# xqz-u/contrast-gan-3D

Measured on NVIDIA B200. Metric: patch_pairs_per_sec_gd_train_step, higher is better.
Workload: dtype bf16

## Files before the change

### contrast_gan_3d_b200/csrc/conv_tc_prog.cu

```cuda
#include "conv_tc_prog_kernel.cuh"

namespace cg {

extern template int prog_launch_ks<1>(ProgPlan &, const ProgLaunchArgs &);
extern template int prog_launch_ks<2>(ProgPlan &, const ProgLaunchArgs &);
extern template int prog_launch_ks<4>(ProgPlan &, const ProgLaunchArgs &);
extern template int prog_launch_ks<8>(ProgPlan &, const ProgLaunchArgs &);

__global__ void repack_prog_kernel(const bf16 *__restrict__ wp, bf16 *__restrict__ wb, int Cb, int Cs, int scatter,
                                   const __grid_constant__ ProgPlan p) {
  const int K = p.paired ? 16 : p.Cin, N = p.Nmma, nh = p.pair ? 2 : 1, Nl = N / nh;
  const int64_t total = (int64_t)p.nbt * K * N;
  for (int64_t i = blockIdx.x * (int64_t)blockDim.x + threadIdx.x; i < total; i += (int64_t)gridDim.x * blockDim.x) {
    const int c8 = (int)(i & 7);
    int64_t t = i >> 3;
    const int nl = (int)(t % Nl); t /= Nl;
    const int cc = (int)(t % (K >> 3)); t /= (K >> 3);
    const int tile = (int)(t % p.nbt);
    const int n = (int)(t / p.nbt) * Nl + nl;
    const int nn = p.stack ? n % p.N : n;
    const int tap = p.stack ? p.tile_phase_tap[tile][n / p.N] : (p.paired ? p.tile_tap[tile][cc] : tile);
    const int ci = p.paired ? c8 : cc * 8 + c8;
    bf16 v = __float2bfloat16_rn(0.f);
    if (nn < p.Nout && tap >= 0) {
// ... 113 lines not shown
            if (nt >= kMaxTaps) return false;
            ProgTap T{};
            T.row_shift = (uint16_t)((oy - offmin) * p.Zh + (oz - offmin));
            T.btile = (uint8_t)nt;
            T.acc = 0; T.first = first ? 1 : 0;
            first = false;
            for (int ph = 0; ph < 8; ++ph) p.tile_phase_tap[nt][ph] = taps8[ph];
            p.taps[nt++] = T; E.ntaps++;
          }
        if (E.ntaps == 0) continue;
        if (ne >= kMaxEntries) return false;
        p.entries[ne++] = E;
      }
      p.nacc = 8;
      p.nentries = ne;
      p.ntaps = nt;
      return true;
    }
    bool seen[8] = {false, false, false, false, false, false, false, false};
    for (int xo = offmin; xo <= offmax; ++xo) {
      ProgEntry E{};
      E.cx = (int8_t)xo; E.cy = (int8_t)offmin; E.cz = (int8_t)offmin;
      E.tap0 = (uint8_t)nt; E.ntaps = 0;
      for (int px = 0; px < 2; ++px)
        for (int dx = 0; dx < k; ++dx) {
          if (((px + 1 - dx) & 1) || (px + 1 - dx) / 2 != xo) continue;
          for (int py = 0; py < 2; ++py)
            for (int dy = 0; dy < k; ++dy) {
              if ((py + 1 - dy) & 1) continue;
              for (int pz = 0; pz < 2; ++pz)
                for (int dz = 0; dz < k; ++dz) {
                  if ((pz + 1 - dz) & 1) continue;
                  if (nt >= kMaxTaps) return false;
                  const int oy = (py + 1 - dy) / 2, oz = (pz + 1 - dz) / 2;
                  ProgTap T{};
                  T.row_shift = (uint16_t)((oy - offmin) * p.Zh + (oz - offmin));
                  T.btile = (uint8_t)((dx * k + dy) * k + dz);
                  T.acc = (uint8_t)((px * 2 + py) * 2 + pz);
                  T.first = seen[T.acc] ? 0 : 1;
                  seen[T.acc] = true;
                  p.taps[nt++] = T; E.ntaps++;
                }
            }
        }
      if (E.ntaps == 0) continue;
      if (ne >= kMaxEntries) return false;
      p.entries[ne++] = E;
    }
    p.nacc = 8;
  }
  p.nentries = ne;
  p.ntaps = nt;
  return true;
}

static bool plan_prog_split(const cgan3d_conv_geom &g, int scatter, ProgPlan &best, int nsplit);

static bool plan_prog(const cgan3d_conv_geom &g, int scatter, ProgPlan &best, int *nsplit_out = nullptr) {
  for (int ns = 1; ns <= 4; ns *= 2)
    if (plan_prog_split(g, scatter, best, ns)) {
      if (nsplit_out) *nsplit_out = ns;
      return true;
    }
  return false;
}

static bool plan_prog_split(const cgan3d_conv_geom &g, int scatter, ProgPlan &best, int nsplit) {
  if (g.stride != 2 || g.pad != 1 || (g.k != 3 && g.k != 4)) return false;
  const int Cin = scatter ? g.Cs : g.Cb, Nfull = scatter ? g.Cb : g.Cs;
  if (Nfull % nsplit || (nsplit > 1 && (Nfull / nsplit) % 16)) return false;
  const int Nout = Nfull / nsplit;
  const int paired = (!scatter && Cin == 8) ? 1 : 0;
  if (!paired && Cin != 16 && Cin != 32 && Cin != 64 && Cin != 128) return false;
  if (Nout % 8 || Nout < 8 || Nout > 256 || (Nout > 8 && Nout % 16)) return false;
  const int N = Nout < 16 ? 16 : Nout;
  const int nacc = scatter ? 8 : 1;
  if (scatter && (g.Xb > 2 * g.Xs || g.Yb > 2 * g.Ys || g.Zb > 2 * g.Zs)) return false;
  const int halo = (scatter && g.k == 4) ? 2 : 1;
  const int taps = g.k * g.k * g.k;
  ProgPlan p{};
  p.B = g.B; p.Xg = g.Xs; p.Yg = g.Ys; p.Zg = g.Zs;
  p.Xo = scatter ? g.Xb : g.Xs; p.Yo = scatter ? g.Yb : g.Ys; p.Zo = scatter ? g.Zb : g.Zs;
  p.Cin = Cin; p.N = N; p.nacc = nacc; p.Nout = Nout; p.paired = paired; p.out_pitch = Nfull; p.out_c0 = 0;
  p.in_scale = scatter ? 1 : 2; p.out_scale = scatter ? 2 : 1;
  p.nbt = paired ? taps / 2 + (g.k == 3 ? 9 : 0) : taps;
  p.btile_bytes = (uint32_t)(paired ? 16 : Cin) * N * 2;
  p.Nmma = N; p.acc_stride = 0; p.mt_stride = N;
  const bool pair_base = paired || Cin <= 64;
  p.pair = (pair_base && N % 32 == 0) ? 1 : 0;
  if (p.pair) p.btile_bytes /= 2;
  if (scatter && 8 * N <= 256) {
    const int ncombo = g.k == 3 ? 8 : 27;
    const uint32_t tile = (uint32_t)Cin * 8 * N * 2 / (pair_base ? 2 : 1);
    if ((ncombo * tile + 1023) / 1024 * 1024 + 40000 <= kSmemLimitProg) {
      p.stack = 1; p.Nmma = 8 * N; p.nbt = ncombo; p.btile_bytes = tile; p.pair = pair_base ? 1 : 0;
    }
  }
  const uint32_t b_total = (p.nbt * p.btile_bytes + 1023) / 1024 * 1024;
  if (b_total + 40000 > kSmemLimitProg) return false;
  const bool zpair = !scatter && !paired && (Cin == 16 || Cin == 32) && g.k == 3 && g.Zb % 2 == 0;
  p.zpair = zpair ? 1 : 0;
  const int a_swz = zpair ? 4 * Cin : ((!paired && Cin <= 64) ? 2 * Cin : 0);
  double best_score = 0;
  bool found = false;
  for (int nzt = 1; nzt <= 4; ++nzt) {
    const int Zt = (p.Zg + nzt - 1) / nzt, Zh = Zt + halo;
    if (2 * (Zh - 1) + 1 > 256) continue;
    for (int Yt = 1; Yt <= p.Yg; ++Yt) {
      const int Yh = Yt + halo;
      if (2 * (Yh - 1) + 1 > 256) break;
      const int mt = (Yt * Zh + 127) / 128;
      if (mt > 4 || 2 * nacc * mt * N > 512) break;
      const int rows_alloc = ((mt * 128 + halo * Zh + halo) + 7) / 8 * 8;
      if (rows_alloc > 16383 || Yh * Zh > rows_alloc) continue;
      const uint32_t slot = a_swz ? ((uint32_t)rows_alloc * a_swz + 1023) / 1024 * 1024 : (uint32_t)(paired ? 1 : Cin / 8) * rows_alloc * 16;
      const int nslots = (int)mn<uint32_t>(8, (kSmemLimitProg - b_total - 512) / slot);
      if (nslots < 3) break;
      const int nslabs = (p.Yg + Yt - 1) / Yt;
      const double eff = (double)p.Yg * p.Zg / ((double)nslabs * nzt * mt * 128);
      const double halo_cost = (double)(Yh * Zh) / (Yt * Zt);
      const double score = eff / (0.5 + 0.5 * halo_cost);
      if (score > best_score + 1e-9) {
        best_score = score; found = true;
        best = p;
        best.nzt = nzt; best.Zt = Zt; best.Zh = Zh; best.Yt = Yt; best.Yh = Yh; best.nslabs = nslabs; best.mtiles = mt;
        best.rows_alloc = rows_alloc; best.slot_bytes = slot; best.nslots = nslots;
      }
    }
  }
  if (!found) return false;
  ProgPlan &q = best;
  const int es = q.in_scale;
  q.a_swz = a_swz;
  if (q.stack) { q.acc_stride = q.N; q.mt_stride = 8 * q.N; }
  else { q.acc_stride = q.mtiles * q.N; q.mt_stride = q.N; }
  q.box_bytes = (a_swz ? (uint32_t)a_swz : 16u) * q.Zh * q.Yh;
  (void)es;
  uint32_t cols = 32;
  while (cols < (uint32_t)(2 * nacc * q.mtiles * N)) cols <<= 1;
  q.tmem_cols = cols;
  q.smem_bytes = b_total + q.nslots * q.slot_bytes + 512;
  q.a_lbo_bytes = paired ? 16u : (uint32_t)q.rows_alloc * 16;
  if (!build_program(g, scatter, q)) return false;
  if (paired || q.stack) {
    if ((uint32_t)q.ntaps * q.btile_bytes > b_total) return false;
    q.nbt = q.ntaps;
  }
  return true;
}

bool tc_prog_supported(const cgan3d_conv_geom &g, int dtype, int op) {
  if (dtype != CGAN3D_BF16 || (op != 0 && op != 1)) return false;
  ProgPlan p;
  return plan_prog(g, op, p);
}

size_t tc_prog_workspace_bytes(const cgan3d_conv_geom &g, int dtype, int op) {
  if (dtype != CGAN3D_BF16 || (op != 0 && op != 1)) return 0;
  ProgPlan p;
  int nsplit = 1;
  if (!plan_prog(g, op, p, &nsplit)) return 0;
  return (((size_t)p.nbt * p.btile_bytes * (p.pair ? 2 : 1) + 255) / 256 * 256) * nsplit + 256;
}

bool tc_prog_fuses_bnstats(const cgan3d_conv_geom &g, int scatter) {
  ProgPlan p;
  return plan_prog(g, scatter, p) && p.Nout <= 64;
}

int tc_prog_run(const cgan3d_conv_geom &g, int scatter, const void *in, const void *wp, void *outp, void *ws, size_t ws_bytes,
                cudaStream_t st, double *bn_sums) {
  ProgPlan p;
  int nsplit = 1;
  if (!plan_prog(g, scatter, p, &nsplit)) return fail(CGAN3D_E_UNSUPPORTED, "tcgen05 strided conv: no tiling for this shape");
  const size_t part_bytes = ((size_t)p.nbt * p.btile_bytes * (p.pair ? 2 : 1) + 255) / 256 * 256;
  const size_t need = part_bytes * nsplit;
  if (ws == nullptr || ws_bytes < need) return fail(CGAN3D_E_WORKSPACE, "tcgen05 strided conv: workspace %zu < %zu", ws_bytes, need);
  if ((reinterpret_cast<uintptr_t>(in) & 15) || (reinterpret_cast<uintptr_t>(outp) & 15) || (reinterpret_cast<uintptr_t>(ws) & 15))
    return fail(CGAN3D_E_ARG, "tcgen05 strided conv: pointers must be 16-byte aligned");
  EncodeTiledFn enc = tc_encode_fn();
  if (!enc) return fail(CGAN3D_E_UNSUPPORTED, "cuTensorMapEncodeTiled not available");
  const int Xi = scatter ? g.Xs : g.Xb, Yi = scatter ? g.Ys : g.Yb, Zi = scatter ? g.Zs : g.Zb, Ci = p.Cin;
  if ((reinterpret_cast<uintptr_t>(outp) & 15) || (p.Nout * 2) % 16 || (p.out_pitch * 2) % 16) return fail(CGAN3D_E_ARG, "tcgen05 strided conv: output rows must be 16-byte aligned");
  const int es = p.in_scale;
  CUtensorMap tm;
  const cuuint64_t zp = p.zpair ? 2 : 1;
  const cuuint64_t gdim[5] = {(cuuint64_t)Ci * zp, (cuuint64_t)Zi / zp, (cuuint64_t)Yi, (cuuint64_t)Xi, (cuuint64_t)g.B};
  const cuuint64_t gstr[4] = {(cuuint64_t)Ci * 2 * zp, (cuuint64_t)Zi * Ci * 2, (cuuint64_t)Yi * Zi * Ci * 2,
                              (cuuint64_t)Xi * Yi * Zi * Ci * 2};
  const cuuint32_t box[5] = {(cuuint32_t)(p.a_swz ? Ci * (int)zp : 8), (cuuint32_t)(p.zpair ? p.Zh : es * (p.Zh - 1) + 1),
                             (cuuint32_t)(es * (p.Yh - 1) + 1), 1, 1};
  const cuuint32_t estr[5] = {1, (cuuint32_t)(p.zpair ? 1 : es), (cuuint32_t)es, 1, 1};
  const CUtensorMapSwizzle swz = p.a_swz == 128 ? CU_TENSOR_MAP_SWIZZLE_128B
                                 : (p.a_swz == 64 ? CU_TENSOR_MAP_SWIZZLE_64B : (p.a_swz == 32 ? CU_TENSOR_MAP_SWIZZLE_32B : CU_TENSOR_MAP_SWIZZLE_NONE));
  CUresult r = enc(&tm, CU_TENSOR_MAP_DATA_TYPE_BFLOAT16, 5, const_cast<void *>(in), gdim, gstr, box, estr,
                   CU_TENSOR_MAP_INTERLEAVE_NONE, swz, CU_TENSOR_MAP_L2_PROMOTION_L2_128B, CU_TENSOR_MAP_FLOAT_OOB_FILL_NONE);
  if (r != CUDA_SUCCESS) return fail(CGAN3D_E_SHAPE, "cuTensorMapEncodeTiled (strided) failed with %d", (int)r);
  const long long total = (long long)p.B * p.nzt * p.nslabs * p.Xg;
  const int grid = p.pair ? 2 * (int)mn<long long>((total + 1) / 2, (long long)(num_sms() / 2)) : (int)mn<long long>(total, (long long)num_sms());
  if (bn_sums && p.Nout > 64) return fail(CGAN3D_E_UNSUPPORTED, "tcgen05 strided conv: fused BatchNorm statistics need <= 64 channels per launch");
  ProgLaunchArgs la{};
  la.tm = tm; la.g = g; la.scatter = scatter; la.nsplit = nsplit; la.grid = grid; la.wp = wp; la.outp = outp; la.ws = ws;
  la.part_bytes = part_bytes; la.bn_sums = bn_sums; la.st = st; la.enc = enc;
  switch (p.paired ? 1 : (p.Cin >> 4)) {
    case 1: return prog_launch_ks<1>(p, la);
    case 2: return prog_launch_ks<2>(p, la);
    case 4: return prog_launch_ks<4>(p, la);
    case 8: return prog_launch_ks<8>(p, la);
    default: return fail(CGAN3D_E_UNSUPPORTED, "tcgen05 strided conv: Cin must be 16, 32, 64 or 128");
  }
}

}
```

### contrast_gan_3d_b200/csrc/conv_tc_prog_kernel.cuh

```cuda
#pragma once
#include "common.cuh"
#include "conv_internal.cuh"
#include "tc_common.cuh"

namespace cg {

using bf16 = __nv_bfloat16;

constexpr int kMaxEntries = 16, kMaxTaps = 64;
constexpr uint32_t kSmemLimitProg = 232448 - 1024;

struct ProgTap {
  uint16_t row_shift;
  uint8_t btile;
  uint8_t acc;
  uint8_t first;
  uint8_t khalf;
  uint8_t pad[2];
};
struct ProgEntry {
  int8_t cx, cy, cz;
  uint8_t ntaps, tap0;
  uint8_t pad[3];
};
struct ProgPlan {
  int B, Xg, Yg, Zg;
  int Xo, Yo, Zo;
  int Cin, N, nacc;
  int Nout;
  int out_pitch, out_c0;
  int paired;
  uint32_t a_lbo_bytes;
  int a_swz;
  int in_scale;
  int out_scale;
  int Zt, nzt, Zh, Yt, nslabs, Yh;
  int mtiles, rows_alloc, nslots, nbt;
  int nentries, ntaps;
  uint32_t slot_bytes, btile_bytes, box_bytes, tmem_cols, smem_bytes;
  ProgEntry entries[kMaxEntries];
  ProgTap taps[kMaxTaps];
  int8_t tile_tap[kMaxTaps][2];
  int stack;
  int Nmma;
  int acc_stride, mt_stride;
  int8_t tile_phase_tap[kMaxTaps][8];
  int pair;
  int zpair;
};

template <int KSTEPS, int MT, int STATS, bool PAIR>
__global__ void __launch_bounds__(192, 1)
conv_prog_tc_kernel(const __grid_constant__ CUtensorMap tmA, const __grid_constant__ CUtensorMap tmW, const bf16 *__restrict__ wB,
                    bf16 *__restrict__ out, const __grid_constant__ ProgPlan p, double *__restrict__ bn_sums) {
  extern __shared__ __align__(1024) uint8_t smem[];
  uint8_t *bres = smem;
  uint8_t *ring = bres + (((size_t)p.nbt * p.btile_bytes + 1023) & ~(size_t)1023);
  uint64_t *bars = reinterpret_cast<uint64_t *>(ring + (size_t)p.nslots * p.slot_bytes);
  uint64_t *b_ready = bars, *s_full = bars + 1, *s_empty = s_full + p.nslots;
  uint64_t *tm_full = s_empty + p.nslots, *tm_empty = tm_full + 2;
  uint32_t *tmem_ptr = reinterpret_cast<uint32_t *>(tm_empty + 2);
  const int warp = threadIdx.x >> 5, lane = threadIdx.x & 31;

  if (threadIdx.x == 0) {
    tc::mbar_init(b_ready, 1);
    for (int i = 0; i < p.nslots; ++i) { tc::mbar_init(&s_full[i], 1); tc::mbar_init(&s_empty[i], 1); }
    for (int i = 0; i < 2; ++i) { tc::mbar_init(&tm_full[i], 1); tc::mbar_init(&tm_empty[i], PAIR ? 8 : 4); }
    tc::fence_barrier_init();
  }
  const uint32_t cta_rank = PAIR ? tc::cluster_ctarank() : 0u;
  if constexpr (PAIR) {
    __syncthreads();
    tc::cluster_sync();
  }
  if (warp == 5) {
    if constexpr (PAIR) { tc::tmem_alloc2(tmem_ptr, p.tmem_cols); tc::tmem_relinquish2(); }
    else { tc::tmem_alloc(tmem_ptr, p.tmem_cols); tc::tmem_relinquish(); }
  }
  tc::tc_fence_before();
  __syncthreads();
  if constexpr (PAIR) tc::cluster_sync();
  tc::tc_fence_after();
  const uint32_t tmem_base = *tmem_ptr;

  const long long total_steps = (long long)p.B * p.nzt * p.nslabs * p.Xg;
  const long long total = PAIR ? (total_steps + 1) / 2 : total_steps;
  const int nblk = PAIR ? (int)gridDim.x >> 1 : (int)gridDim.x, blk = PAIR ? (int)blockIdx.x >> 1 : (int)blockIdx.x;
  const int s_begin = (int)(total * blk / nblk), s_end = (int)(total * (blk + 1) / nblk);
  const int kch = (p.paired || p.a_swz) ? 1 : (p.Cin >> 3);
  auto decode = [&](int st, int &b, int &z0, int &zlen, int &y0, int &ylen, int &x) -> bool {
    bool live = true;
    if constexpr (PAIR) {
      st = 2 * st + (int)cta_rank;
      if (st >= total_steps) { st = (int)total_steps - 1; live = false; }
    }
    x = st % p.Xg; st /= p.Xg;
    const int sl = st % p.nslabs; st /= p.nslabs;
    const int zt = st % p.nzt;
    b = st / p.nzt;
    y0 = sl * p.Yt; ylen = min(p.Yt, p.Yg - y0);
    z0 = zt * p.Zt; zlen = min(p.Zt, p.Zg - z0);
    return live;
  };

  if (warp == 4) {
    if (lane == 0) {
      tc::tma_prefetch_desc(&tmA);
      if constexpr (PAIR) {
        tc::tma_prefetch_desc(&tmW);
        if (cta_rank == 0) tc::mbar_expect_tx(b_ready, 2u * (uint32_t)p.nbt * p.btile_bytes);
        const int trows = (int)(p.btile_bytes >> 8);
        for (int t = 0; t < p.nbt; ++t)
          tc::tma_load_2d_2cta(bres + (size_t)t * p.btile_bytes, &tmW, b_ready, 0, ((int)cta_rank * p.nbt + t) * trows);
      } else {
        tc::mbar_expect_tx(b_ready, (uint32_t)p.nbt * p.btile_bytes);
        for (int t = 0; t < p.nbt; ++t)
          tc::bulk_g2s(bres + (size_t)t * p.btile_bytes, reinterpret_cast<const uint8_t *>(wB) + (size_t)t * p.btile_bytes,
                       p.btile_bytes, b_ready);
      }
      uint32_t e = 0;
      for (int st = s_begin; st < s_end; ++st) {
        int b, z0, zlen, y0, ylen, x;
        decode(st, b, z0, zlen, y0, ylen, x);
        for (int en = 0; en < p.nentries; ++en, ++e) {
          const ProgEntry &E = p.entries[en];
          const uint32_t slot = e % p.nslots, use = e / p.nslots;
          if (use > 0) tc::mbar_wait(&s_empty[slot], (use - 1) & 1);
          uint8_t *dst = ring + (size_t)slot * p.slot_bytes;
          const int cz = (p.zpair ? z0 : p.in_scale * z0) + E.cz, cy = p.in_scale * y0 + E.cy, cx = p.in_scale * x + E.cx;
          if constexpr (PAIR) {
            if (cta_rank == 0) tc::mbar_expect_tx(&s_full[slot], 2 * p.box_bytes);
            tc::tma_load_5d_2cta(dst, &tmA, &s_full[slot], 0, cz, cy, cx, b);
            continue;
          }
          tc::mbar_expect_tx(&s_full[slot], p.box_bytes * kch);
          if (p.a_swz) {
            tc::tma_load_5d(dst, &tmA, &s_full[slot], 0, cz, cy, cx, b);
          } else {
            for (int cc = 0; cc < kch; ++cc)
              tc::tma_load_5d(dst + (size_t)cc * p.rows_alloc * 16, &tmA, &s_full[slot], cc * 8, cz, cy, cx, b);
          }
        }
      }
    }
  } else if (warp == 5 && cta_rank != 0) {
  } else if (warp == 5) {
    const bool leader = tc::elect_one();
    const uint32_t idesc = tc::make_idesc_bf16(PAIR ? 256 : 128, p.Nmma, 0, 0);
    const uint32_t ring_u32 = tc::smem_u32(ring), b_u32 = tc::smem_u32(bres);
    const uint32_t a_lbo = p.a_lbo_bytes, b_lbo = (uint32_t)(PAIR ? p.Nmma >> 1 : p.Nmma) * 16;
    auto commit = [&](uint64_t *bar) {
      if constexpr (PAIR) tc::umma_commit_2cta(bar, 3);
      else tc::umma_commit(bar);
    };
    const uint32_t a_row = p.a_swz ? (uint32_t)p.a_swz >> 4 : 1u;
    const uint64_t a_hi = p.a_swz ? tc::make_desc_sw(0, 8u * p.a_swz, (uint32_t)p.a_swz) : tc::make_desc(0, a_lbo, 128);
    const uint64_t b_hi = tc::make_desc(0, b_lbo, 128);
    const uint32_t a_kstep = p.a_swz ? 2u : (2 * a_lbo) >> 4, b_kstep = (2 * b_lbo) >> 4;
    tc::mbar_wait(b_ready, 0);
    tc::tc_fence_after();
    uint32_t e = 0, acc = 0;
    for (int st = s_begin; st < s_end; ++st, ++acc) {
      const uint32_t q = acc & 1, uq = acc >> 1;
      if (uq > 0) tc::mbar_wait(&tm_empty[q], (uq - 1) & 1);
      tc::tc_fence_after();
      const uint32_t d_base = tmem_base + q * (uint32_t)(p.nacc * MT * p.N);
      for (int en = 0; en < p.nentries; ++en, ++e) {
        const ProgEntry &E = p.entries[en];
        const uint32_t slot = e % p.nslots;
        tc::mbar_wait(&s_full[slot], (e / p.nslots) & 1);
        tc::tc_fence_after();
        const uint32_t a_slot = (ring_u32 + slot * p.slot_bytes) >> 4;
        for (int t = 0; t < E.ntaps; ++t) {
          const ProgTap &T = p.taps[E.tap0 + t];
          const uint64_t a0 = a_hi | (uint64_t)((a_slot + T.row_shift * a_row + (uint32_t)T.khalf * (uint32_t)(p.Cin >> 3)) & 0x3FFF);
          const uint64_t b0 = b_hi | (uint64_t)(((b_u32 + (uint32_t)T.btile * p.btile_bytes) >> 4) & 0x3FFF);
          const uint32_t d0 = d_base + (uint32_t)T.acc * p.acc_stride;
          const uint32_t keep = T.first ? 0u : 1u;
          if (leader) {
#pragma unroll
            for (int mt = 0; mt < MT; ++mt) {
#pragma unroll
              for (int kk = 0; kk < KSTEPS; ++kk) {
                if constexpr (PAIR)
                  tc::umma_bf16_2cta(d0 + mt * p.mt_stride, a0 + (uint64_t)(mt * 128 * a_row + kk * a_kstep), b0 + (uint64_t)(kk * b_kstep),
                                     idesc, (kk != 0) ? 1u : keep);
                else
                  tc::umma_bf16(d0 + mt * p.mt_stride, a0 + (uint64_t)(mt * 128 * a_row + kk * a_kstep), b0 + (uint64_t)(kk * b_kstep), idesc,
                                (kk != 0) ? 1u : keep);
              }
            }
          }
          __syncwarp();
        }
        if (leader) commit(&s_empty[slot]);
        __syncwarp();
      }
      if (leader) commit(&tm_full[q]);
      __syncwarp();
    }
  } else {
    uint32_t acc = 0;
    float ssum[STATS ? STATS : 1], ssq[STATS ? STATS : 1];
    if (STATS) {
#pragma unroll
      for (int j = 0; j < STATS; ++j) { ssum[j] = 0.f; ssq[j] = 0.f; }
    }
    for (int st = s_begin; st < s_end; ++st, ++acc) {
      int b, z0, zlen, y0, ylen, x;
      const bool live = decode(st, b, z0, zlen, y0, ylen, x);
      const uint32_t q = acc & 1;
      tc::mbar_wait(&tm_full[q], (acc >> 1) & 1);
      tc::tc_fence_after();
      const uint32_t d_base = tmem_base + ((uint32_t)(warp * 32) << 16) + q * (uint32_t)(p.nacc * MT * p.N);
      auto emit = [&](const uint32_t (&v)[16], int a, int mt, auto cc_tag) {
        constexpr int cc = decltype(cc_tag)::value;
        const int px = (a >> 2) & 1, py = (a >> 1) & 1, pz = a & 1;
        const int ox = p.out_scale * x + px;
        const int r = mt * 128 + warp * 32 + lane;
        const int gy = r / p.Zh, gz = r - gy * p.Zh;
        const int oy = p.out_scale * (y0 + gy) + py, oz = p.out_scale * (z0 + gz) + pz;
        if (!(live && gy < ylen && gz < zlen && ox < p.Xo && oy < p.Yo && oz < p.Zo)) return;
        bf16 *dst = out + ((((size_t)b * p.Xo + ox) * p.Yo + oy) * p.Zo + oz) * p.out_pitch + p.out_c0 + cc * 16;
        uint32_t pk[8];
#pragma unroll
        for (int j = 0; j < 8; ++j) {
          __nv_bfloat162 h = __floats2bfloat162_rn(__uint_as_float(v[2 * j]), __uint_as_float(v[2 * j + 1]));
          pk[j] = *reinterpret_cast<uint32_t *>(&h);
        }
        uint4 *d4 = reinterpret_cast<uint4 *>(dst);
        if (cc * 16 + 8 < p.Nout && (p.out_pitch & 15) == 0 && (reinterpret_cast<uintptr_t>(out) & 31) == 0) {
          tc::st_global_v8(dst, pk);
        } else {
          d4[0] = make_uint4(pk[0], pk[1], pk[2], pk[3]);
          if (cc * 16 + 8 < p.Nout) d4[1] = make_uint4(pk[4], pk[5], pk[6], pk[7]);
        }
        if constexpr (STATS > cc * 16) {
#pragma unroll
          for (int j = 0; j < 16; ++j) {
            const float f = __uint_as_float(v[j]);
            ssum[cc * 16 + j] += f;
            ssq[cc * 16 + j] += f * f;
          }
        }
      };
      for (int mt = 0; mt < MT; ++mt) {
        const uint32_t t_mt = d_base + (uint32_t)(mt * p.mt_stride);
        if (p.nacc == 1) {
          uint32_t v[4][16];
          if (0 < p.Nout) tc::tmem_ld16(t_mt + 0, v[0]);
          if (16 < p.Nout) tc::tmem_ld16(t_mt + 16, v[1]);
          if (32 < p.Nout) tc::tmem_ld16(t_mt + 32, v[2]);
          if (48 < p.Nout) tc::tmem_ld16(t_mt + 48, v[3]);
          tc::tmem_ld_wait();
          if (0 < p.Nout) emit(v[0], 0, mt, std::integral_constant<int, 0>{});
          if (16 < p.Nout) emit(v[1], 0, mt, std::integral_constant<int, 1>{});
          if (32 < p.Nout) emit(v[2], 0, mt, std::integral_constant<int, 2>{});
          if (48 < p.Nout) emit(v[3], 0, mt, std::integral_constant<int, 3>{});
          if constexpr (STATS == 0) {
            for (int c0 = 64; c0 < p.Nout; c0 += 16) {
              tc::tmem_ld16(t_mt + c0, v[0]);
              tc::tmem_ld_wait();
              const int r = mt * 128 + warp * 32 + lane;
              const int gy = r / p.Zh, gz = r - gy * p.Zh;
              if (live && gy < ylen && gz < zlen && x < p.Xo && y0 + gy < p.Yo && z0 + gz < p.Zo) {
                bf16 *dst = out + ((((size_t)b * p.Xo + x) * p.Yo + (y0 + gy)) * p.Zo + (z0 + gz)) * p.out_pitch + p.out_c0 + c0;
                uint32_t pk[8];
#pragma unroll
                for (int j = 0; j < 8; ++j) {
                  __nv_bfloat162 h = __floats2bfloat162_rn(__uint_as_float(v[0][2 * j]), __uint_as_float(v[0][2 * j + 1]));
                  pk[j] = *reinterpret_cast<uint32_t *>(&h);
                }
                if ((p.out_pitch & 15) == 0 && (reinterpret_cast<uintptr_t>(out) & 31) == 0) {
                  tc::st_global_v8(dst, pk);
                } else {
                  uint4 *d4 = reinterpret_cast<uint4 *>(dst);
                  d4[0] = make_uint4(pk[0], pk[1], pk[2], pk[3]);
                  d4[1] = make_uint4(pk[4], pk[5], pk[6], pk[7]);
                }
              }
            }
          }
        } else {
          auto phases4 = [&](auto cc_tag) {
            constexpr int cc = decltype(cc_tag)::value;
            if (cc * 16 >= p.Nout) return;
#pragma unroll
            for (int g = 0; g < 2; ++g) {
              uint32_t v[4][16];
#pragma unroll
              for (int j = 0; j < 4; ++j) tc::tmem_ld16(t_mt + (uint32_t)((4 * g + j) * p.acc_stride + cc * 16), v[j]);
              tc::tmem_ld_wait();
#pragma unroll
              for (int j = 0; j < 4; ++j) emit(v[j], 4 * g + j, mt, cc_tag);
            }
          };
          phases4(std::integral_constant<int, 0>{});
          phases4(std::integral_constant<int, 1>{});
          phases4(std::integral_constant<int, 2>{});
          phases4(std::integral_constant<int, 3>{});
        }
      }
      tc::tc_fence_before();
      __syncwarp();
      if (lane == 0) {
        if constexpr (PAIR) tc::mbar_arrive_cluster(&tm_empty[q], 0);
        else tc::mbar_arrive(&tm_empty[q]);
      }
    }
    if constexpr (STATS > 0) {
      float r0[64], r1[64];
#pragma unroll
      for (int j = 0; j < 64; ++j) { r0[j] = j < STATS ? ssum[j < STATS ? j : 0] : 0.f; r1[j] = j < STATS ? ssq[j < STATS ? j : 0] : 0.f; }
      warp_reduce64(r0, lane);
      warp_reduce64(r1, lane);
      const int ch = warp_reduce64_channel(lane);
#pragma unroll
      for (int i = 0; i < 2; ++i)
        if (ch + i < p.Nout) {
          atomicAdd(&bn_sums[p.out_c0 + ch + i], (double)r0[i]);
          atomicAdd(&bn_sums[p.out_pitch + p.out_c0 + ch + i], (double)r1[i]);
        }
    }
  }
  tc::tc_fence_before();
  __syncthreads();
  if constexpr (PAIR) {
    tc::cluster_sync();
    if (warp == 5) tc::tmem_dealloc2(tmem_base, p.tmem_cols);
  } else {
    if (warp == 5) tc::tmem_dealloc(tmem_base, p.tmem_cols);
  }
}

int repack_prog_launch(const bf16 *wp, bf16 *wb, int Cb, int Cs, int scatter, const ProgPlan &p, cudaStream_t st);

struct ProgLaunchArgs {
  CUtensorMap tm;
  cgan3d_conv_geom g;
  int scatter, nsplit, grid;
  const void *wp;
  void *outp, *ws;
  size_t part_bytes;
  double *bn_sums;
  cudaStream_t st;
  EncodeTiledFn enc;
};

template <int KS_>
int prog_launch_ks(ProgPlan &p, const ProgLaunchArgs &a) {
  const CUtensorMap &tm = a.tm;
  const cgan3d_conv_geom &g = a.g;
  const int scatter = a.scatter, nsplit = a.nsplit, grid = a.grid;
  const void *wp = a.wp;
  void *outp = a.outp, *ws = a.ws;
  const size_t part_bytes = a.part_bytes;
  double *bn_sums = a.bn_sums;
  cudaStream_t st = a.st;
  EncodeTiledFn enc = a.enc;
  auto launch_s = [&](auto ks_tag, auto mt_tag, auto st_tag, auto pair_tag) -> int {
    constexpr int KS = decltype(ks_tag)::value;
    constexpr int MT = decltype(mt_tag)::value;
    constexpr int ST = decltype(st_tag)::value;
    constexpr bool PR = decltype(pair_tag)::value;
    static bool attr_set = false;
    if (!attr_set) {
      cudaError_t e = cudaFuncSetAttribute(conv_prog_tc_kernel<KS, MT, ST, PR>, cudaFuncAttributeMaxDynamicSharedMemorySize,
                                           (int)kSmemLimitProg + 1024);
      if (e != cudaSuccess) return cuda_fail(e, "cudaFuncSetAttribute(conv_prog_tc_kernel)");
      attr_set = true;
    }
    for (int part = 0; part < nsplit; ++part) {
      p.out_c0 = part * p.Nout;
      bf16 *wb = reinterpret_cast<bf16 *>(reinterpret_cast<uint8_t *>(ws) + part * part_bytes);
      if (int rr = repack_prog_launch(reinterpret_cast<const bf16 *>(wp), wb, g.Cb, g.Cs, scatter, p, st)) return rr;
      CUtensorMap tmw{};
      if (PR) {
        const cuuint64_t wdim[2] = {64, (cuuint64_t)2 * p.nbt * (p.btile_bytes >> 8)};
        const cuuint64_t wstr[1] = {256};
        const cuuint32_t wbox[2] = {64, (cuuint32_t)(p.btile_bytes >> 8)};
        const cuuint32_t we[2] = {1, 1};
        CUresult rw = enc(&tmw, CU_TENSOR_MAP_DATA_TYPE_INT32, 2, wb, wdim, wstr, wbox, we, CU_TENSOR_MAP_INTERLEAVE_NONE,
                          CU_TENSOR_MAP_SWIZZLE_NONE, CU_TENSOR_MAP_L2_PROMOTION_L2_128B, CU_TENSOR_MAP_FLOAT_OOB_FILL_NONE);
// ... 51 lines not shown
```

### contrast_gan_3d_b200/csrc/wgrad_s2_tc.cu

```cuda
#include "common.cuh"
#include "conv_internal.cuh"
#include "tc_common.cuh"

namespace cg {

using bf16 = __nv_bfloat16;
constexpr uint32_t kSmemLimitWs = 232448 - 2048;
constexpr int kMaxWsMma = 4;

struct WsPlan {
  int B, X, Y, Z;
  int Cb, Cs, k, taps;
  int Zh, Yt, Yh, nslabs;
  int kpad, rowsA, rowsB;
  int stride;
  int nsrc, nblkB;
  uint32_t lboB;
  int nmma, stages, steps_per_dx;
  uint16_t row_shift[kMaxWsMma];
  int8_t acc_tap[kMaxWsMma][2][4];
  uint32_t rowbytesA, rowbytesB, a_bytes, srcB_bytes, stage_bytes, boxA_bytes, boxB_bytes, smem_bytes, tmem_cols;
  int m128;
};

__global__ void __launch_bounds__(192, 1)
wgrad_s2_sw_kernel(const __grid_constant__ CUtensorMap tmY, const __grid_constant__ CUtensorMap tmX, float *__restrict__ dw,
                   const __grid_constant__ WsPlan p) {
  extern __shared__ __align__(1024) uint8_t smem_raw[];
  uint8_t *stage_mem = reinterpret_cast<uint8_t *>((reinterpret_cast<uintptr_t>(smem_raw) + 1023) & ~(uintptr_t)1023);
  uint64_t *bars = reinterpret_cast<uint64_t *>(stage_mem + (size_t)p.stages * p.stage_bytes);
  uint64_t *full = bars, *empty = bars + p.stages, *done = bars + 2 * p.stages;
  uint32_t *tmem_ptr = reinterpret_cast<uint32_t *>(done + 1);
  const int warp = threadIdx.x >> 5, lane = threadIdx.x & 31;

  {
    uint4 *z = reinterpret_cast<uint4 *>(stage_mem);
    const uint32_t n16 = (uint32_t)p.stages * p.stage_bytes / 16;
    for (uint32_t i = threadIdx.x; i < n16; i += blockDim.x) z[i] = make_uint4(0, 0, 0, 0);
  }
  if (threadIdx.x == 0) {
    for (int i = 0; i < p.stages; ++i) { tc::mbar_init(&full[i], 1); tc::mbar_init(&empty[i], 1); }
    tc::mbar_init(done, 1);
    tc::fence_barrier_init();
  }
  if (warp == 5) {
    tc::tmem_alloc(tmem_ptr, p.tmem_cols);
    tc::tmem_relinquish();
  }
  tc::fence_proxy_async();
  tc::tc_fence_before();
  __syncthreads();
  tc::tc_fence_after();
  const uint32_t tmem_base = *tmem_ptr;

  const int dx = blockIdx.x % p.k;
  const int grp = blockIdx.x / p.k, ngrp = (gridDim.x - dx + p.k - 1) / p.k;
  const int s_begin = (int)((long long)p.steps_per_dx * grp / ngrp), s_end = (int)((long long)p.steps_per_dx * (grp + 1) / ngrp);
  const int ncol = p.nblkB * p.Cb;

  if (warp == 4) {
    if (lane == 0) {
      tc::tma_prefetch_desc(&tmY);
      tc::tma_prefetch_desc(&tmX);
      for (int st = s_begin, n = 0; st < s_end; ++st, ++n) {
        int t = st;
        const int x = t % p.X; t /= p.X;
        const int sl = t % p.nslabs;
        const int b = t / p.nslabs;
        const int y0 = sl * p.Yt;
        const uint32_t s = n % p.stages, use = n / p.stages;
        if (use > 0) tc::mbar_wait(&empty[s], (use - 1) & 1);
        tc::mbar_expect_tx(&full[s], p.boxA_bytes + p.nsrc * p.boxB_bytes);
        uint8_t *a = stage_mem + (size_t)s * p.stage_bytes, *bb = a + p.a_bytes;
        tc::tma_load_5d(a, &tmY, &full[s], 0, -1, y0, x, b);
        if (p.stride == 2) {
          for (int src = 0; src < 4; ++src)
            tc::tma_load_5d(bb + (size_t)src * p.srcB_bytes, &tmX, &full[s], 0, -(src & 1), 2 * y0 - (src >> 1), 2 * x + dx - 1, b);
        } else {
          tc::tma_load_5d(bb, &tmX, &full[s], 0, -1, y0 - 1, x + dx - 1, b);
        }
      }
    }
  } else if (warp == 5) {
    const bool leader = tc::elect_one();
    const uint32_t idesc = tc::make_idesc_bf16(p.m128 ? 128 : 64, ncol, 1, 1);
    const uint64_t a_hi = tc::make_desc_sw_mn(0, p.rowbytesA, 8 * p.rowbytesA, p.rowbytesA);
    const uint64_t b_hi = tc::make_desc_sw_mn(0, p.lboB, 8 * p.rowbytesB, p.rowbytesB);
    const uint32_t stage0 = tc::smem_u32(stage_mem);
    const int kblocks = p.kpad >> 4;
    const uint32_t a_step = (16 * p.rowbytesA) >> 4, b_step = (16 * p.rowbytesB) >> 4;
    for (int st = s_begin, n = 0; st < s_end; ++st, ++n) {
      const uint32_t s = n % p.stages;
      tc::mbar_wait(&full[s], (n / p.stages) & 1);
      tc::tc_fence_after();
      const uint32_t a0 = (stage0 + s * p.stage_bytes) >> 4, b0 = (stage0 + s * p.stage_bytes + p.a_bytes) >> 4;
      if (leader) {
        for (int j = 0; j < p.nmma; ++j) {
          const uint32_t d = p.m128 ? tmem_base + (uint32_t)(j * ncol) : tmem_base + (uint32_t)((j >> 1) * ncol) + ((uint32_t)((j & 1) * 16) << 16);
          uint64_t a_desc = a_hi | (uint64_t)(a0 & 0x3FFF);
          uint64_t b_desc = b_hi | (uint64_t)((b0 + ((uint32_t)p.row_shift[j] * p.rowbytesB >> 4)) & 0x3FFF);
          tc::umma_bf16(d, a_desc, b_desc, idesc, n != 0 ? 1u : 0u);
#pragma unroll 4
          for (int kb = 1; kb < kblocks; ++kb) {
            a_desc += a_step;
            b_desc += b_step;
            tc::umma_bf16(d, a_desc, b_desc, idesc, 1u);
          }
        }
        tc::umma_commit(&empty[s]);
      }
      __syncwarp();
    }
    if (leader) tc::umma_commit(done);
    __syncwarp();
  } else if (s_end > s_begin) {
    tc::mbar_wait(done, 0);
    tc::tc_fence_after();
    float *dw_dx = dw + dx * p.k * p.k;
    if (p.m128) {
      const int m = warp * 32 + lane;
      const int cs = m & 63, blk = m >> 6;
      for (int j = 0; j < p.nmma; ++j)
        for (int c0 = 0; c0 < ncol; c0 += 16) {
          uint32_t v[16];
          tc::tmem_ld16(tmem_base + ((uint32_t)(warp * 32) << 16) + (uint32_t)(j * ncol + c0), v);
          tc::tmem_ld_wait();
#pragma unroll
          for (int c = 0; c < 16; ++c) {
            const int nn = c0 + c;
            const int src = nn / p.Cb, cb = nn - src * p.Cb;
            const int t2 = p.acc_tap[j][blk][src];
            if (t2 >= 0) atomicAdd(&dw_dx[((size_t)cs * p.Cb + cb) * p.taps + t2], __uint_as_float(v[c]));
          }
        }
    } else {
    const int m = warp * 16 + (lane & 15);
    const int cs = m % p.Cs, blk = m / p.Cs;
    const int ngroups = (p.nmma + 1) >> 1;
    for (int g2 = 0; g2 < ngroups; ++g2) {
      const int j = g2 * 2 + (lane >> 4);
      for (int c0 = 0; c0 < ncol; c0 += 16) {
        uint32_t v[16];
        tc::tmem_ld16(tmem_base + ((uint32_t)(warp * 32) << 16) + (uint32_t)(g2 * ncol + c0), v);
        tc::tmem_ld_wait();
        if (j < p.nmma) {
#pragma unroll
          for (int c = 0; c < 16; ++c) {
            const int nn = c0 + c;
            const int src = nn / p.Cb, cb = nn - src * p.Cb;
            const int t2 = p.acc_tap[j][blk][src];
            if (t2 >= 0) atomicAdd(&dw_dx[((size_t)cs * p.Cb + cb) * p.taps + t2], __uint_as_float(v[c]));
          }
        }
      }
    }
    }
  }
  tc::tc_fence_before();
  __syncthreads();
  if (warp == 5) tc::tmem_dealloc(tmem_base, p.tmem_cols);
}

static bool plan_ws(const cgan3d_conv_geom &g, WsPlan &p) {
  const int k = g.k, s = g.stride;
  if (g.pad != 1) return false;
  if (s == 2) {
    if (k != 3 && k != 4) return false;
    if (g.Cs != 32 && g.Cs != 64) return false;
    if (g.Cb != 16 && g.Cb != 32) return false;
  } else if (s == 1) {
    if (k != 3 || g.Cs != 64) return false;
    if (g.Cb != 16 && g.Cb != 32 && g.Cb != 64) return false;
    if (g.Xb != g.Xs || g.Yb != g.Ys || g.Zb != g.Zs) return false;
  } else {
    return false;
  }
  p = WsPlan{};
  p.B = g.B; p.X = g.Xs; p.Y = g.Ys; p.Z = g.Zs; p.Cb = g.Cb; p.Cs = g.Cs; p.k = k; p.taps = k * k * k;
  p.stride = s;
  const int halo = s == 1 ? 2 : 1;
  p.Zh = p.Z + halo;
  if (s * (p.Zh - 1) + 1 > 256) return false;
  p.m128 = g.Cs == 64 ? 1 : 0;
  p.rowbytesA = 2u * g.Cs;
  p.rowbytesB = 2u * g.Cb;
  p.stages = 2;
  int nm = 0;
  if (s == 2) {
    p.nsrc = 4; p.nblkB = 4;
    auto cls = [](int d) { return (d - 1) & 1; };
    auto shf = [&](int d) { return (d - 1 + cls(d)) / 2; };
    auto find = [&](int c, int sh) { for (int d = 0; d < k; ++d) if (cls(d) == c && shf(d) == sh) return d; return -1; };
    for (int by = 0; by < 2; ++by) {
      bool any = false;
// ... 112 lines not shown
```

Before: 911.1.

## Stage scatter epilogue through swizzled smem for coalesced stores; incremental step decode

For the stride-2 transposed (scatter) conv path, the epilogue now converts each pair of z-phase accumulators to bf16, writes them into a per-warp swizzled shared-memory staging buffer, then reissues them as lane-cooperative 16-byte stores so adjacent z outputs land contiguously. This targets the scattered, poorly coalesced global writes of the old per-phase emit. Reserving staging smem can lower the number of ring slots. Step index decoding and ring slot/phase tracking in the conv and wgrad kernels also move from per-iteration div/mod to incremental counters.

```diff
diff --git a/contrast_gan_3d_b200/csrc/conv_tc_prog.cu b/contrast_gan_3d_b200/csrc/conv_tc_prog.cu
--- a/contrast_gan_3d_b200/csrc/conv_tc_prog.cu
+++ b/contrast_gan_3d_b200/csrc/conv_tc_prog.cu
@@ -219,7 +219,7 @@
   p.B = g.B; p.Xg = g.Xs; p.Yg = g.Ys; p.Zg = g.Zs;
   p.Xo = scatter ? g.Xb : g.Xs; p.Yo = scatter ? g.Yb : g.Ys; p.Zo = scatter ? g.Zb : g.Zs;
   p.Cin = Cin; p.N = N; p.nacc = nacc; p.Nout = Nout; p.paired = paired; p.out_pitch = Nfull; p.out_c0 = 0;
-  p.in_scale = scatter ? 1 : 2; p.out_scale = scatter ? 2 : 1;
+  p.in_scale = scatter ? 1 : 2;
   p.nbt = paired ? taps / 2 + (g.k == 3 ? 9 : 0) : taps;
   p.btile_bytes = (uint32_t)(paired ? 16 : Cin) * N * 2;
   p.Nmma = N; p.acc_stride = 0; p.mt_stride = N;
@@ -236,6 +236,7 @@
   const uint32_t b_total = (p.nbt * p.btile_bytes + 1023) / 1024 * 1024;
   if (b_total + 40000 > kSmemLimitProg) return false;
   const bool zpair = !scatter && !paired && (Cin == 16 || Cin == 32) && g.k == 3 && g.Zb % 2 == 0;
+  const uint32_t stage = scatter ? 4u * 32 * 64 : 0u;
   p.zpair = zpair ? 1 : 0;
   const int a_swz = zpair ? 4 * Cin : ((!paired && Cin <= 64) ? 2 * Cin : 0);
   double best_score = 0;
@@ -251,7 +252,7 @@
       const int rows_alloc = ((mt * 128 + halo * Zh + halo) + 7) / 8 * 8;
       if (rows_alloc > 16383 || Yh * Zh > rows_alloc) continue;
       const uint32_t slot = a_swz ? ((uint32_t)rows_alloc * a_swz + 1023) / 1024 * 1024 : (uint32_t)(paired ? 1 : Cin / 8) * rows_alloc * 16;
-      const int nslots = (int)mn<uint32_t>(8, (kSmemLimitProg - b_total - 512) / slot);
+      const int nslots = (int)mn<uint32_t>(8, (kSmemLimitProg - b_total - 512 - stage) / slot);
       if (nslots < 3) break;
       const int nslabs = (p.Yg + Yt - 1) / Yt;
       const double eff = (double)p.Yg * p.Zg / ((double)nslabs * nzt * mt * 128);
@@ -276,7 +277,8 @@
   uint32_t cols = 32;
   while (cols < (uint32_t)(2 * nacc * q.mtiles * N)) cols <<= 1;
   q.tmem_cols = cols;
-  q.smem_bytes = b_total + q.nslots * q.slot_bytes + 512;
+  q.stage_bytes = stage;
+  q.smem_bytes = b_total + q.nslots * q.slot_bytes + stage + 512;
   q.a_lbo_bytes = paired ? 16u : (uint32_t)q.rows_alloc * 16;
   if (!build_program(g, scatter, q)) return false;
   if (paired || q.stack) {
diff --git a/contrast_gan_3d_b200/csrc/conv_tc_prog_kernel.cuh b/contrast_gan_3d_b200/csrc/conv_tc_prog_kernel.cuh
--- a/contrast_gan_3d_b200/csrc/conv_tc_prog_kernel.cuh
+++ b/contrast_gan_3d_b200/csrc/conv_tc_prog_kernel.cuh
@@ -33,7 +33,6 @@
   uint32_t a_lbo_bytes;
   int a_swz;
   int in_scale;
-  int out_scale;
   int Zt, nzt, Zh, Yt, nslabs, Yh;
   int mtiles, rows_alloc, nslots, nbt;
   int nentries, ntaps;
@@ -47,6 +46,7 @@
   int8_t tile_phase_tap[kMaxTaps][8];
   int pair;
   int zpair;
+  uint32_t stage_bytes;
 };
 
 template <int KSTEPS, int MT, int STATS, bool PAIR>
@@ -56,7 +56,8 @@
   extern __shared__ __align__(1024) uint8_t smem[];
   uint8_t *bres = smem;
   uint8_t *ring = bres + (((size_t)p.nbt * p.btile_bytes + 1023) & ~(size_t)1023);
-  uint64_t *bars = reinterpret_cast<uint64_t *>(ring + (size_t)p.nslots * p.slot_bytes);
+  uint8_t *stage = ring + (size_t)p.nslots * p.slot_bytes;
+  uint64_t *bars = reinterpret_cast<uint64_t *>(stage + p.stage_bytes);
   uint64_t *b_ready = bars, *s_full = bars + 1, *s_empty = s_full + p.nslots;
   uint64_t *tm_full = s_empty + p.nslots, *tm_empty = tm_full + 2;
   uint32_t *tmem_ptr = reinterpret_cast<uint32_t *>(tm_empty + 2);
@@ -88,19 +89,35 @@
   const int nblk = PAIR ? (int)gridDim.x >> 1 : (int)gridDim.x, blk = PAIR ? (int)blockIdx.x >> 1 : (int)blockIdx.x;
   const int s_begin = (int)(total * blk / nblk), s_end = (int)(total * (blk + 1) / nblk);
   const int kch = (p.paired || p.a_swz) ? 1 : (p.Cin >> 3);
-  auto decode = [&](int st, int &b, int &z0, int &zlen, int &y0, int &ylen, int &x) -> bool {
-    bool live = true;
+  struct StepPos {
+    int x, sl, zt, b;
+    bool live;
+  };
+  auto step_first = [&](int st) -> StepPos {
+    StepPos s;
+    s.live = true;
     if constexpr (PAIR) {
       st = 2 * st + (int)cta_rank;
-      if (st >= total_steps) { st = (int)total_steps - 1; live = false; }
-    }
-    x = st % p.Xg; st /= p.Xg;
-    const int sl = st % p.nslabs; st /= p.nslabs;
-    const int zt = st % p.nzt;
-    b = st / p.nzt;
-    y0 = sl * p.Yt; ylen = min(p.Yt, p.Yg - y0);
-    z0 = zt * p.Zt; zlen = min(p.Zt, p.Zg - z0);
-    return live;
+      if (st >= total_steps) { st = (int)total_steps - 1; s.live = false; }
+    }
+    s.x = st % p.Xg; st /= p.Xg;
+    s.sl = st % p.nslabs; st /= p.nslabs;
+    s.zt = st % p.nzt;
+    s.b = st / p.nzt;
+    return s;
+  };
+  auto step_next = [&](StepPos &s, int st_next) {
+    if constexpr (PAIR) {
+      if (2LL * st_next + (long long)cta_rank >= total_steps) { s = step_first(st_next); return; }
+    }
+    s.x += PAIR ? 2 : 1;
+    while (s.x >= p.Xg) {
+      s.x -= p.Xg;
+      if (++s.sl == p.nslabs) {
+        s.sl = 0;
+        if (++s.zt == p.nzt) { s.zt = 0; ++s.b; }
+      }
+    }
   };
 
   if (warp == 4) {
@@ -118,27 +135,29 @@
           tc::bulk_g2s(bres + (size_t)t * p.btile_bytes, reinterpret_cast<const uint8_t *>(wB) + (size_t)t * p.btile_bytes,
                        p.btile_bytes, b_ready);
       }
-      uint32_t e = 0;
-      for (int st = s_begin; st < s_end; ++st) {
-        int b, z0, zlen, y0, ylen, x;
-        decode(st, b, z0, zlen, y0, ylen, x);
-        for (int en = 0; en < p.nentries; ++en, ++e) {
+      uint32_t slot = 0, ephase = 0;
+      bool first_lap = true;
+      StepPos sp = step_first(s_begin);
+      for (int st = s_begin; st < s_end; step_next(sp, ++st)) {
+        const int x = sp.x, y0 = sp.sl * p.Yt, z0 = sp.zt * p.Zt, b = sp.b;
+        for (int en = 0; en < p.nentries; ++en) {
           const ProgEntry &E = p.entries[en];
-          const uint32_t slot = e % p.nslots, use = e / p.nslots;
-          if (use > 0) tc::mbar_wait(&s_empty[slot], (use - 1) & 1);
+          if (!first_lap) tc::mbar_wait(&s_empty[slot], ephase ^ 1);
           uint8_t *dst = ring + (size_t)slot * p.slot_bytes;
+          const uint32_t cur = slot;
+          if (++slot == (uint32_t)p.nslots) { slot = 0; ephase ^= 1; first_lap = false; }
           const int cz = (p.zpair ? z0 : p.in_scale * z0) + E.cz, cy = p.in_scale * y0 + E.cy, cx = p.in_scale * x + E.cx;
           if constexpr (PAIR) {
-            if (cta_rank == 0) tc::mbar_expect_tx(&s_full[slot], 2 * p.box_bytes);
-            tc::tma_load_5d_2cta(dst, &tmA, &s_full[slot], 0, cz, cy, cx, b);
+            if (cta_rank == 0) tc::mbar_expect_tx(&s_full[cur], 2 * p.box_bytes);
+            tc::tma_load_5d_2cta(dst, &tmA, &s_full[cur], 0, cz, cy, cx, b);
             continue;
           }
-          tc::mbar_expect_tx(&s_full[slot], p.box_bytes * kch);
+          tc::mbar_expect_tx(&s_full[cur], p.box_bytes * kch);
           if (p.a_swz) {
-            tc::tma_load_5d(dst, &tmA, &s_full[slot], 0, cz, cy, cx, b);
+            tc::tma_load_5d(dst, &tmA, &s_full[cur], 0, cz, cy, cx, b);
           } else {
             for (int cc = 0; cc < kch; ++cc)
-              tc::tma_load_5d(dst + (size_t)cc * p.rows_alloc * 16, &tmA, &s_full[slot], cc * 8, cz, cy, cx, b);
+              tc::tma_load_5d(dst + (size_t)cc * p.rows_alloc * 16, &tmA, &s_full[cur], cc * 8, cz, cy, cx, b);
           }
         }
       }
@@ -159,16 +178,15 @@
     const uint32_t a_kstep = p.a_swz ? 2u : (2 * a_lbo) >> 4, b_kstep = (2 * b_lbo) >> 4;
     tc::mbar_wait(b_ready, 0);
     tc::tc_fence_after();
-    uint32_t e = 0, acc = 0;
+    uint32_t slot = 0, sphase = 0, acc = 0;
     for (int st = s_begin; st < s_end; ++st, ++acc) {
       const uint32_t q = acc & 1, uq = acc >> 1;
       if (uq > 0) tc::mbar_wait(&tm_empty[q], (uq - 1) & 1);
       tc::tc_fence_after();
       const uint32_t d_base = tmem_base + q * (uint32_t)(p.nacc * MT * p.N);
-      for (int en = 0; en < p.nentries; ++en, ++e) {
+      for (int en = 0; en < p.nentries; ++en) {
         const ProgEntry &E = p.entries[en];
-        const uint32_t slot = e % p.nslots;
-        tc::mbar_wait(&s_full[slot], (e / p.nslots) & 1);
+        tc::mbar_wait(&s_full[slot], sphase);
         tc::tc_fence_after();
         const uint32_t a_slot = (ring_u32 + slot * p.slot_bytes) >> 4;
         for (int t = 0; t < E.ntaps; ++t) {
@@ -195,6 +213,7 @@
         }
         if (leader) commit(&s_empty[slot]);
         __syncwarp();
+        if (++slot == (uint32_t)p.nslots) { slot = 0; sphase ^= 1; }
       }
       if (leader) commit(&tm_full[q]);
       __syncwarp();
@@ -206,20 +225,21 @@
 #pragma unroll
       for (int j = 0; j < STATS; ++j) { ssum[j] = 0.f; ssq[j] = 0.f; }
     }
-    for (int st = s_begin; st < s_end; ++st, ++acc) {
-      int b, z0, zlen, y0, ylen, x;
-      const bool live = decode(st, b, z0, zlen, y0, ylen, x);
+    uint4 *stage_w = reinterpret_cast<uint4 *>(stage) + warp * 128;
+    StepPos sp = step_first(s_begin);
+    for (int st = s_begin; st < s_end; step_next(sp, ++st), ++acc) {
+      const int x = sp.x, b = sp.b, y0 = sp.sl * p.Yt, z0 = sp.zt * p.Zt;
+      const int ylen = min(p.Yt, p.Yg - y0), zlen = min(p.Zt, p.Zg - z0);
+      const bool live = sp.live;
       const uint32_t q = acc & 1;
       tc::mbar_wait(&tm_full[q], (acc >> 1) & 1);
       tc::tc_fence_after();
       const uint32_t d_base = tmem_base + ((uint32_t)(warp * 32) << 16) + q * (uint32_t)(p.nacc * MT * p.N);
-      auto emit = [&](const uint32_t (&v)[16], int a, int mt, auto cc_tag) {
+      auto emit = [&](const uint32_t (&v)[16], int mt, auto cc_tag) {
         constexpr int cc = decltype(cc_tag)::value;
-        const int px = (a >> 2) & 1, py = (a >> 1) & 1, pz = a & 1;
-        const int ox = p.out_scale * x + px;
         const int r = mt * 128 + warp * 32 + lane;
         const int gy = r / p.Zh, gz = r - gy * p.Zh;
-        const int oy = p.out_scale * (y0 + gy) + py, oz = p.out_scale * (z0 + gz) + pz;
+        const int ox = x, oy = y0 + gy, oz = z0 + gz;
         if (!(live && gy < ylen && gz < zlen && ox < p.Xo && oy < p.Yo && oz < p.Zo)) return;
         bf16 *dst = out + ((((size_t)b * p.Xo + ox) * p.Yo + oy) * p.Zo + oz) * p.out_pitch + p.out_c0 + cc * 16;
         uint32_t pk[8];
@@ -253,10 +273,10 @@
           if (32 < p.Nout) tc::tmem_ld16(t_mt + 32, v[2]);
           if (48 < p.Nout) tc::tmem_ld16(t_mt + 48, v[3]);
           tc::tmem_ld_wait();
-          if (0 < p.Nout) emit(v[0], 0, mt, std::integral_constant<int, 0>{});
-          if (16 < p.Nout) emit(v[1], 0, mt, std::integral_constant<int, 1>{});
-          if (32 < p.Nout) emit(v[2], 0, mt, std::integral_constant<int, 2>{});
-          if (48 < p.Nout) emit(v[3], 0, mt, std::integral_constant<int, 3>{});
+          if (0 < p.Nout) emit(v[0], mt, std::integral_constant<int, 0>{});
+          if (16 < p.Nout) emit(v[1], mt, std::integral_constant<int, 1>{});
+          if (32 < p.Nout) emit(v[2], mt, std::integral_constant<int, 2>{});
+          if (48 < p.Nout) emit(v[3], mt, std::integral_constant<int, 3>{});
           if constexpr (STATS == 0) {
             for (int c0 = 64; c0 < p.Nout; c0 += 16) {
               tc::tmem_ld16(t_mt + c0, v[0]);
@@ -282,23 +302,64 @@
             }
           }
         } else {
-          auto phases4 = [&](auto cc_tag) {
-            constexpr int cc = decltype(cc_tag)::value;
-            if (cc * 16 >= p.Nout) return;
-#pragma unroll
-            for (int g = 0; g < 2; ++g) {
-              uint32_t v[4][16];
-#pragma unroll
-              for (int j = 0; j < 4; ++j) tc::tmem_ld16(t_mt + (uint32_t)((4 * g + j) * p.acc_stride + cc * 16), v[j]);
+          const int r = mt * 128 + warp * 32 + lane;
+          const int gy = r / p.Zh, gz = r - gy * p.Zh;
+          const int oz = 2 * (z0 + gz);
+          const bool row_ok = live && gy < ylen && gz < zlen;
+          const int hv = p.Nout >= 16 ? 2 : 1;
+          const int rsh = hv == 2 ? 2 : 1;
+          const size_t pz_stride = (size_t)p.out_pitch * 2;
+#pragma unroll 1
+          for (int pxy = 0; pxy < 4; ++pxy) {
+            const int ox = 2 * x + (pxy >> 1), oy = 2 * (y0 + gy) + (pxy & 1);
+            const int zv = (row_ok && ox < p.Xo && oy < p.Yo) ? min(2, p.Zo - oz) : 0;
+            const unsigned long long base = reinterpret_cast<unsigned long long>(
+                out + ((((size_t)b * p.Xo + ox) * p.Yo + oy) * p.Zo + oz) * p.out_pitch + p.out_c0);
+            auto chunk = [&](auto cc_tag) {
+              constexpr int cc = decltype(cc_tag)::value;
+              if (cc * 16 >= p.Nout) return;
+              uint32_t v[2][16];
+              tc::tmem_ld16(t_mt + (uint32_t)((2 * pxy) * p.acc_stride + cc * 16), v[0]);
+              tc::tmem_ld16(t_mt + (uint32_t)((2 * pxy + 1) * p.acc_stride + cc * 16), v[1]);
               tc::tmem_ld_wait();
-#pragma unroll
-              for (int j = 0; j < 4; ++j) emit(v[j], 4 * g + j, mt, cc_tag);
-            }
-          };
-          phases4(std::integral_constant<int, 0>{});
-          phases4(std::integral_constant<int, 1>{});
-          phases4(std::integral_constant<int, 2>{});
-          phases4(std::integral_constant<int, 3>{});
+              __syncwarp();
+#pragma unroll
+              for (int pz = 0; pz < 2; ++pz) {
+                uint32_t pk[8];
+#pragma unroll
+                for (int j = 0; j < 8; ++j) {
+                  __nv_bfloat162 h = __floats2bfloat162_rn(__uint_as_float(v[pz][2 * j]), __uint_as_float(v[pz][2 * j + 1]));
+                  pk[j] = *reinterpret_cast<uint32_t *>(&h);
+                }
+                const int sw = (lane >> 1) & 3;
+                stage_w[lane * 4 + ((2 * pz) ^ sw)] = make_uint4(pk[0], pk[1], pk[2], pk[3]);
+                stage_w[lane * 4 + ((2 * pz + 1) ^ sw)] = make_uint4(pk[4], pk[5], pk[6], pk[7]);
+                if constexpr (STATS > cc * 16) {
+                  if (pz < zv) {
+#pragma unroll
+                    for (int j = 0; j < 16; ++j) {
+                      const float f = __uint_as_float(v[pz][j]);
+                      ssum[cc * 16 + j] += f;
+                      ssq[cc * 16 + j] += f * f;
+                    }
+                  }
+                }
+              }
+              __syncwarp();
+#pragma unroll
+              for (int it = 0; it < 4; ++it) {
+                if (it >= 2 * hv) break;
+                const int row = (it << (5 - rsh)) + (lane >> rsh), u = lane & ((1 << rsh) - 1);
+                const int pz = u >> (hv - 1), half = u & (hv - 1);
+                const unsigned long long d_row = __shfl_sync(0xffffffffu, base, row);
+                const int zv_row = __shfl_sync(0xffffffffu, zv, row);
+                const uint4 val = stage_w[row * 4 + ((2 * pz + half) ^ ((row >> 1) & 3))];
+                if (pz < zv_row) reinterpret_cast<uint4 *>(d_row + pz * pz_stride + cc * 32)[half] = val;
+              }
+            };
+            chunk(std::integral_constant<int, 0>{});
+            chunk(std::integral_constant<int, 1>{});
+          }
         }
       }
       tc::tc_fence_before();
diff --git a/contrast_gan_3d_b200/csrc/wgrad_s2_tc.cu b/contrast_gan_3d_b200/csrc/wgrad_s2_tc.cu
--- a/contrast_gan_3d_b200/csrc/wgrad_s2_tc.cu
+++ b/contrast_gan_3d_b200/csrc/wgrad_s2_tc.cu
@@ -62,14 +62,12 @@
     if (lane == 0) {
       tc::tma_prefetch_desc(&tmY);
       tc::tma_prefetch_desc(&tmX);
-      for (int st = s_begin, n = 0; st < s_end; ++st, ++n) {
-        int t = st;
-        const int x = t % p.X; t /= p.X;
-        const int sl = t % p.nslabs;
-        const int b = t / p.nslabs;
+      int x = s_begin % p.X, sl = (s_begin / p.X) % p.nslabs, b = s_begin / (p.X * p.nslabs);
+      uint32_t s = 0, phase = 0;
+      bool first_lap = true;
+      for (int st = s_begin; st < s_end; ++st) {
         const int y0 = sl * p.Yt;
-        const uint32_t s = n % p.stages, use = n / p.stages;
-        if (use > 0) tc::mbar_wait(&empty[s], (use - 1) & 1);
+        if (!first_lap) tc::mbar_wait(&empty[s], phase ^ 1);
         tc::mbar_expect_tx(&full[s], p.boxA_bytes + p.nsrc * p.boxB_bytes);
         uint8_t *a = stage_mem + (size_t)s * p.stage_bytes, *bb = a + p.a_bytes;
         tc::tma_load_5d(a, &tmY, &full[s], 0, -1, y0, x, b);
@@ -79,6 +77,11 @@
         } else {
           tc::tma_load_5d(bb, &tmX, &full[s], 0, -1, y0 - 1, x + dx - 1, b);
         }
+        if (++s == (uint32_t)p.stages) { s = 0; phase ^= 1; first_lap = false; }
+        if (++x == p.X) {
+          x = 0;
+          if (++sl == p.nslabs) { sl = 0; ++b; }
+        }
       }
     }
   } else if (warp == 5) {
@@ -89,9 +92,9 @@
     const uint32_t stage0 = tc::smem_u32(stage_mem);
     const int kblocks = p.kpad >> 4;
     const uint32_t a_step = (16 * p.rowbytesA) >> 4, b_step = (16 * p.rowbytesB) >> 4;
+    uint32_t s = 0, phase = 0;
     for (int st = s_begin, n = 0; st < s_end; ++st, ++n) {
-      const uint32_t s = n % p.stages;
-      tc::mbar_wait(&full[s], (n / p.stages) & 1);
+      tc::mbar_wait(&full[s], phase);
       tc::tc_fence_after();
       const uint32_t a0 = (stage0 + s * p.stage_bytes) >> 4, b0 = (stage0 + s * p.stage_bytes + p.a_bytes) >> 4;
       if (leader) {
@@ -110,6 +113,7 @@
         tc::umma_commit(&empty[s]);
       }
       __syncwarp();
+      if (++s == (uint32_t)p.stages) { s = 0; phase ^= 1; }
     }
     if (leader) tc::umma_commit(done);
     __syncwarp();
```

Result: no change. 914.4, median of 6 (+0.4%).
